# talmolab/VNL-Brax-Imitation

Measured on AMD Instinct MI355X. Metric: env-steps/sec (whole node), rodent imitation, num_envs=4096/GPU, higher is better.
Workload: dtype f32; 1 GPU; rodent imitation rollout, single groom clip, 4096 envs/GPU: intention-policy forward (HIP) -> RodentTracking.step (5 substeps, CG 6/6) -> auto-reset on -> Transition logging (unroll 20, the 20 steps replayed as one captured hipGraph); envs_per_gpu=4096, clips=1, parallelism=env-sharded x1, no data-path collective

## Files before the change

__graft_entry__.py:

```python
from __future__ import annotations

import os
import sys

ROOT = os.path.dirname(os.path.abspath(__file__))
if ROOT not in sys.path:
    sys.path.insert(0, ROOT)


def build() -> None:
    import vnl_brax_imitation_amd
    from vnl_brax_imitation_amd.csrc import build as hip_build

    from concurrent.futures import ThreadPoolExecutor

    with ThreadPoolExecutor(5) as pool:
        futs = {v: pool.submit(hip_build.build, variant=v) for v in ("product", "spill", "noblk", "nospec", "tail")}
        paths = {v: f.result() for v, f in futs.items()}
    path = paths["product"]
    assert all(os.path.exists(p_) for p_ in paths.values()), paths
    from oracle import oracle as _oracle

    _oracle.build()
    from vnl_brax_imitation_amd import _lib

    _lib.load_library(path)
    print(f"[build] {path} ok; oracle ok")


def smoke() -> None:
    import numpy as np
    import torch

    sys.path.insert(0, os.path.join(ROOT, "tests"))
    import helpers as H
    from vnl_brax_imitation_amd.envs.rodent import RodentTracking

    assert torch.cuda.is_available(), "smoke() needs a HIP device"
    B = 256
    env = RodentTracking(H.reference_clip(), num_envs=B, device="cuda:0", **H.env_kwargs())
    rng = np.random.default_rng(0)
    sf = rng.integers(0, 235, B).astype(np.int32)
    noise = (1e-3 * rng.standard_normal((B, 74))).astype(np.float32)
    st = env.reset(start_frame=torch.from_numpy(sf), noise=torch.from_numpy(noise))
    act = np.clip(0.3 * rng.standard_normal((B, 30)), -1, 1).astype(np.float32)
    o = H.make_oracle(env, "f64")
    ost = o.env_reset(sf, noise)
    e_reset = H.scaled_err(st.pipeline_state.qacc_warmstart.cpu().numpy(), ost["qacc_warmstart"])
    e_obs = H.scaled_err(st.obs.cpu().numpy(), ost["obs"])
    import parity as P
# ... 33 lines not shown
```

vnl-brax-imitation_amd/csrc/build.py:

```python
from __future__ import annotations

import os
import subprocess
import sys

HERE = os.path.dirname(os.path.abspath(__file__))
SOURCES = ["vnl_lib.hip", "vnl_policy.hip", "vnl_ppo.hip", "vnl_domain.hip"]
DEPS = SOURCES + ["vnl_env_kernels.h", "vnl_body.h", "vnl_types.h", "vnl_policy_train.h", "../../include/vnl.h"]
OUT = os.path.join(HERE, "libvnl.so")

VARIANTS = {
    "product": ("libvnl.so", ["-DVNL_KERNEL_ATTR=__attribute__((amdgpu_waves_per_eu(2,2)))"]),
    "prof": ("libvnl_prof.so", ["-DVNL_PROFILE", "-DVNL_KERNEL_ATTR=__attribute__((amdgpu_waves_per_eu(2,2)))"]),
    "knobs": ("libvnl_knobs.so", ["-DVNL_STAGE_KNOBS", "-DVNL_KERNEL_ATTR=__attribute__((amdgpu_waves_per_eu(2,2)))"]),
    "spill": ("libvnl_spill.so", ["-DVNL_KERNEL_ATTR=__attribute__((amdgpu_waves_per_eu(4,4)))"]),
    "noblk": ("libvnl_noblk.so", ["-DVNL_NO_BLK", "-DVNL_KERNEL_ATTR=__attribute__((amdgpu_waves_per_eu(2,2)))"]),
    "tail": ("libvnl_tail.so", ["-DVNL_SOLVER_TAIL", "-DVNL_KERNEL_ATTR=__attribute__((amdgpu_waves_per_eu(2,2)))"]),
    "nospec": ("libvnl_nospec.so", ["-DVNL_NO_SPEC", "-DVNL_KERNEL_ATTR=__attribute__((amdgpu_waves_per_eu(2,2)))"]),
}
ENV_KERNELS = ("vnl_step_kernel", "vnl_reset_kernel")


def resource_usage(stderr_text: str) -> dict:
    out, name = {}, None
    for line in stderr_text.splitlines():
        if "Function Name:" in line:
            name = line.split("Function Name:")[1].split()[0]
            out[name] = {}
        elif name and "remark:" in line:
            body = line.split("remark:")[1].split("[-Rpass")[0].strip()
            key, _, val = body.rpartition(":")
            try:
                out[name][key.strip()] = int(val.strip())
            except ValueError:
                pass
    return out


def build(force: bool = False, verbose: bool = False, profile: bool = False, knobs: bool = False,
          variant: str | None = None) -> str:
    variant = variant or ("prof" if profile else ("knobs" if knobs else "product"))
    fname, defs = VARIANTS[variant]
    out = os.path.join(HERE, fname)
    deps = [os.path.join(HERE, d) for d in DEPS] + [os.path.abspath(__file__)]
    newest = max(os.path.getmtime(d) for d in deps)
    if not force and os.path.exists(out) and os.path.getmtime(out) >= newest:
        return out
    hipcc = os.environ.get("HIPCC", "/opt/rocm/bin/hipcc")
    objdir = os.path.join(HERE, "_obj", variant)
    os.makedirs(objdir, exist_ok=True)
# ... 68 lines not shown
```

vnl-brax-imitation_amd/csrc/vnl_body.h:

```cpp
#pragma once
#include <math.h>

#include "vnl_types.h"

#ifndef VNL_HD
#define VNL_HD __device__ __forceinline__
#endif

#ifndef VNL_FORKJOIN_DEFINED
#define VNL_LANES 64
#define VNL_ROWS_PER_LANE 8
#define VNL_ROWS_SMALL 5
#define VNL_CHAIN_WIDTH 8
#define VNL_ROWSETS_1 1
#define VNL_ROWSETS_2 2
#define VNL_FOR(i, n) for (int i = (int)lane; i < (n); i += VNL_LANES)
#define VNL_SERIAL if (lane == 0)
#define VNL_SYNC() __builtin_amdgcn_fence(__ATOMIC_ACQ_REL, "wavefront")
#define VNL_SYNC_GLOBAL()                                     \
  do {                                                        \
    __builtin_amdgcn_fence(__ATOMIC_ACQ_REL, "wavefront");    \
    asm volatile("s_waitcnt vmcnt(0)" ::: "memory");          \
    __builtin_amdgcn_fence(__ATOMIC_ACQ_REL, "wavefront");    \
  } while (0)
// ... 123 lines not shown
VNL_HD M3 qmat(Q4 q) {
  M3 m;
  vreal q00 = q.w * q.w, q01 = q.w * q.x, q02 = q.w * q.y, q03 = q.w * q.z;
  vreal q11 = q.x * q.x, q12 = q.x * q.y, q13 = q.x * q.z, q22 = q.y * q.y, q23 = q.y * q.z, q33 = q.z * q.z;
  m.a[0] = q00 + q11 - q22 - q33, m.a[1] = vreal(2.) * (q12 - q03), m.a[2] = vreal(2.) * (q13 + q02);
  m.a[3] = vreal(2.) * (q12 + q03), m.a[4] = q00 - q11 + q22 - q33, m.a[5] = vreal(2.) * (q23 - q01);
  m.a[6] = vreal(2.) * (q13 - q02), m.a[7] = vreal(2.) * (q23 + q01), m.a[8] = q00 - q11 - q22 + q33;
  return m;
}
VNL_HD V3 mmul(const M3& m, V3 v) {
  return V3{m.a[0] * v.x + m.a[1] * v.y + m.a[2] * v.z, m.a[3] * v.x + m.a[4] * v.y + m.a[5] * v.z,
            m.a[6] * v.x + m.a[7] * v.y + m.a[8] * v.z};
}
struct S6 {
  V3 a, l;
};
VNL_HD S6 operator+(S6 p, S6 q) { return S6{p.a + q.a, p.l + q.l}; }
VNL_HD S6 operator*(S6 p, vreal s) { return S6{p.a * s, p.l * s}; }
VNL_HD vreal dot(S6 p, S6 q) { return dot(p.a, q.a) + dot(p.l, q.l); }
VNL_HD S6 mcross(S6 u, S6 v) { return S6{cross(u.a, v.a), cross(u.l, v.a) + cross(u.a, v.l)}; }
VNL_HD S6 mcross_force(S6 v, S6 f) { return S6{cross(v.a, f.a) + cross(v.l, f.l), cross(v.a, f.l)}; }

#if defined(__HIP_DEVICE_COMPILE__)
#define VNL_CAS __attribute__((address_space(4)))
#define VNL_TO_CAS(T, p) ((const VNL_CAS T*)(unsigned long long)(p))
#define VNL_LAUNDER(p) asm volatile("" : "+s"(p))
#else
#define VNL_CAS
#define VNL_TO_CAS(T, p) ((const T*)(p))
#define VNL_LAUNDER(p)
#endif
#define MI(f) (SP::fixed ? SP::D.f : m.f)
#define LO(f) (SP::fixed ? SP::L.f : L.f)
template <class SP>
struct EnvWaveT {
  const VNL_CAS DevModel& m;
  const VNL_CAS DevEnv& ev;
  const DevState& st;
  const VNL_CAS WsLayout& L;
  vreal* s;
  unsigned e, lane;
  const VNL_CAS KernelConsts* kc;
  int* trace;
  VNL_HD EnvWaveT with_trace(int* t) const { return EnvWaveT{m, ev, st, L, s, e, lane, kc, t}; }
  VNL_HD EnvWaveT fresh() const {
    const VNL_CAS KernelConsts* k = kc;
    VNL_LAUNDER(k);
    return EnvWaveT{k->m, k->ev, st, k->L, s, e, lane, k, trace};
  }
#ifdef VNL_PROFILE
  VNL_HD void prof_begin() const {
    if (lane == 0) {
      for (int i = 0; i < VNL_NPROF; i++) s[LO(prof) + i] = 0.f;
      s[LO(prof) + VNL_NPROF] = __builtin_bit_cast(float, (unsigned)__builtin_amdgcn_s_memtime());
    }
  }
  VNL_HD void prof_end() const {
    if (lane == 0)
      for (int i = 0; i < VNL_NPROF; i++) atomicAdd(&g_vnl_prof[i], (unsigned long long)s[LO(prof) + i]);
  }
#else
  VNL_HD void prof_begin() const {}
  VNL_HD void prof_end() const {}
#endif

  VNL_HD V3 ld3(int o) const { return V3{s[o], s[o + 1], s[o + 2]}; }
  VNL_HD void st3(int o, V3 v) const { s[o] = v.x, s[o + 1] = v.y, s[o + 2] = v.z; }
  VNL_HD Q4 ld4(int o) const { return Q4{s[o], s[o + 1], s[o + 2], s[o + 3]}; }
  VNL_HD S6 ld6(int o) const { return S6{ld3(o), ld3(o + 3)}; }
  VNL_HD void st6(int o, S6 v) const { st3(o, v.a), st3(o + 3, v.l); }
  VNL_HD static V3 t3(const vreal* t, int i) { return V3{t[3 * i], t[3 * i + 1], t[3 * i + 2]}; }
  VNL_HD static Q4 t4(const vreal* t, int i) { return Q4{t[4 * i], t[4 * i + 1], t[4 * i + 2], t[4 * i + 3]}; }

  VNL_HD S6 inert_mul(int o, S6 v) const {
    vreal ixx = s[o], iyy = s[o + 1], izz = s[o + 2], ixy = s[o + 3], ixz = s[o + 4], iyz = s[o + 5];
    V3 mp = ld3(o + 6);
    vreal mass = s[o + 9];
    V3 ang = V3{ixx * v.a.x + ixy * v.a.y + ixz * v.a.z, ixy * v.a.x + iyy * v.a.y + iyz * v.a.z,
                ixz * v.a.x + iyz * v.a.y + izz * v.a.z} +
             cross(mp, v.l);
    V3 lin = v.l * mass - cross(mp, v.a);
// ... 43 lines not shown
    const vreal* x = gxpos() + 3 * b;
    return V3{x[0], x[1], x[2]};
  }
  VNL_HD Q4 gquat4(int b) const {
    const vreal* q = gxquat() + 4 * b;
    return Q4{q[0], q[1], q[2], q[3]};
  }
  VNL_HD V3 ref_point() const { return MI(root_free) ? ld3(LO(qpos)) : V3{m.root_px, m.root_py, m.root_pz}; }

  VNL_HD int anc_of(int k) const { return ((const unsigned char*)(s + LO(tab_anc)))[k]; }
  VNL_HD int madr(int d) const { return ((const unsigned short*)(s + LO(tab_madr)))[d]; }
  VNL_HD int eadr(int d) const { return ((const unsigned short*)(s + LO(tab_madr)))[MI(nv) + d]; }
  VNL_HD int depth(int d) const { return eadr(d) - madr(d); }
  VNL_HD int ndesc(int d) const { return ((const unsigned short*)(s + LO(tab_madr)))[2 * MI(nv) + d]; }
  VNL_HD int parent_of(int b) const { return ((const unsigned char*)(s + LO(tab_body)))[b]; }
  VNL_HD int dofadr_of(int b) const { return ((const unsigned char*)(s + LO(tab_body)))[MI(nbody) + b]; }
  VNL_HD int dofnum_of(int b) const { return ((const unsigned char*)(s + LO(tab_body)))[2 * MI(nbody) + b]; }
  VNL_HD int con_body(int c) const { return ((const unsigned char*)(s + LO(tab_body)))[3 * MI(nbody) + c]; }
  VNL_HD unsigned short* live_rows() const { return (unsigned short*)((int*)(s + LO(act_list)) + (MI(ncon) + 3) / 4 + 2); }
  VNL_HD int num_live_rows() const { return ((const int*)(s + LO(act_list)))[(MI(ncon) + 3) / 4 + 1]; }
  template <class F>
  VNL_HD void for_live_rows(F body) const {
    const int nl = num_live_rows();
    if (nl <= VNL_LIVE_MAX) {
      const unsigned short* lv = live_rows();
      VNL_FOR(l, nl) body((int)lv[l]);
    } else {
      VNL_FOR(r, MI(nefc)) body(r);
    }
  }
  VNL_HD int con_lastdof(int c) const { return ((const unsigned char*)(s + LO(tab_body)))[3 * MI(nbody) + MI(ncon) + c]; }
  VNL_HD int lvl_dof(int q) const { return ((const unsigned char*)(s + LO(tab_lvl)))[q]; }
  VNL_HD int lvl_start(int l) const { return ((const unsigned char*)(s + LO(tab_lvl)))[MI(nv) + l]; }
  VNL_HD int jump_of(int r, int b) const { return ((const unsigned char*)(s + LO(tab_jump)))[r * MI(nbody) + b]; }
  VNL_HD void load_tables() const {
    unsigned char* ta = (unsigned char*)(s + LO(tab_anc));
    VNL_FOR(k, MI(nM)) ta[k] = (unsigned char)m.M_anc[k];
    unsigned short* tm = (unsigned short*)(s + LO(tab_madr));
    VNL_FOR(d, MI(nv)) {
      tm[d] = (unsigned short)m.dof_Madr[d], tm[MI(nv) + d] = (unsigned short)(m.dof_Madr[d] + m.dof_depth[d]);
      tm[2 * MI(nv) + d] = (unsigned short)m.dof_ndesc[d];
    }
    unsigned char* tb = (unsigned char*)(s + LO(tab_body));
    VNL_FOR(b, MI(nbody)) {
      tb[b] = (unsigned char)m.body_parent[b];
      tb[MI(nbody) + b] = (unsigned char)m.body_dofadr[b];
      tb[2 * MI(nbody) + b] = (unsigned char)m.body_dofnum[b];
    }
    VNL_FOR(c, MI(ncon)) {
      int cb = m.cg_body[m.con_geom[c] & 0xff];
      tb[3 * MI(nbody) + c] = (unsigned char)cb;
      tb[3 * MI(nbody) + MI(ncon) + c] = (unsigned char)m.body_lastdof[cb];
    }
    unsigned char* tl = (unsigned char*)(s + LO(tab_lvl));
    VNL_FOR(q, MI(nv) + MI(max_depth) + 2) tl[q] = m.lvl_tab[q];
    unsigned char* tj = (unsigned char*)(s + LO(tab_jump));
    VNL_FOR(q, MI(jump_rounds) * MI(nbody)) tj[q] = m.jump[q];
    VNL_SYNC();
  }

  VNL_HD void kinematics() const {
    int A = LO(P), Bf = LO(P) + 7 * MI(nbody);
    auto put_pose = [&](int base, int b, V3 pos, Q4 quat) {
      st3(base + 7 * b, pos);
      s[base + 7 * b + 3] = quat.w, s[base + 7 * b + 4] = quat.x, s[base + 7 * b + 5] = quat.y, s[base + 7 * b + 6] = quat.z;
    };
    auto hinge_chain = [&](int b, V3& pos, Q4& quat) {
      const int jn = m.body_jntnum[b], ja = m.body_jntadr[b];
      for (int k = 0; k < jn; k++) {
        const int j = ja + k, qa = m.jnt_qposadr[j], da = m.jnt_dofadr[j];
        V3 jp = t3(m.jnt_pos, j), jax = t3(m.jnt_axis, j);
        V3 anchor = qrot(jp, quat) + pos;
        st6(LO(cdof) + 6 * da, S6{qrot(jax, quat), anchor});
        vreal ang = s[LO(qpos) + qa] - m.jnt_qpos0[j];
        vreal sn = sin(vreal(0.5) * ang), cs = cos(vreal(0.5) * ang);
        quat = qmul(quat, Q4{cs, jax.x * sn, jax.y * sn, jax.z * sn});
        pos = anchor - qrot(jp, quat);
      }
    };
    VNL_FOR(k, MI(nbody) - 2) {
      const int b = k + 2;
      V3 pos = t3(m.body_pos, b);
      Q4 quat = t4(m.body_quat, b);
      hinge_chain(b, pos, quat);
      put_pose(A, b, pos, quat);
    }
// ... 728 lines not shown
#pragma unroll
        for (int u = 0; u < W; u++) l[u] = ld[ST * e[u]];
        vreal p0 = vreal(0.), p1 = vreal(0.);
#pragma unroll
        for (int u = 0; u < W; u += 2) {
          p0 += i + u <= iend ? l[u] * x[u] : vreal(0.);
          p1 += i + u + 1 <= iend ? l[u + 1] * x[u + 1] : vreal(0.);
        }
        acc += p0 + p1;
      }
      s[out + a] = dmode == 1 ? acc * s[dinvb + ST * a] : (dmode == 2 ? acc / s[dinvb + ST * a] : acc);
    }
    VNL_SYNC();
  }

  template <int ST, bool COL>
  VNL_HD void blk_apply(int in, int out, int dmode, int LDb, int dinvb) const {
    const int cfg = MI(blk_cfg);
    const int trips = COL ? (cfg >> 4) & 15 : cfg & 15, steps = COL ? (cfg >> 12) & 15 : (cfg >> 8) & 15;
    const unsigned* tab = m.blk_tab + (COL ? (cfg & 15) * 64 : 0);
    constexpr int W = VNL_BLK_W, MAXT = 4;
#ifdef __HIP_DEVICE_COMPILE__
    unsigned pre[MAXT];
#pragma unroll
    for (int t = 0; t < MAXT; t++) pre[t] = t < trips ? tab[t * 64 + (int)lane] : 0u;
#endif
#pragma unroll
    for (int trip = 0; trip < MAXT; trip++) {
      if (trip >= trips) break;
      VNL_PERLANE(vreal, part);
      VNL_PERLANE(unsigned, dsc);
      VNL_FOR(l, VNL_WAVE_ITEMS(64)) {
#ifdef __HIP_DEVICE_COMPILE__
        const unsigned d = pre[trip];
#else
        const unsigned d = tab[trip * 64 + l];
#endif
        const int n = (int)(d >> 16) & 15;
        vreal l_[W], x[W];
        if constexpr (!COL) {
          const int e0 = (int)(d & 0xffffu);
          const unsigned char* an = (const unsigned char*)(s + LO(tab_anc)) + e0;
          const vreal* row = s + LDb + ST * e0;
          int j[W];
#pragma unroll
          for (int u = 0; u < W; u++) j[u] = an[u], l_[u] = row[ST * u];
#pragma unroll
          for (int u = 0; u < W; u++) x[u] = s[in + j[u]];
        } else {
          const int i0 = (int)(d & 0x7fu), da = (int)(d >> 7) & 0x3f;
          const unsigned short* ea = (const unsigned short*)(s + LO(tab_madr)) + MI(nv) + i0;
          const vreal* ld = s + LDb - ST * da;
          int e[W];
#pragma unroll
          for (int u = 0; u < W; u++) e[u] = ea[u], x[u] = s[in + i0 + u];
#pragma unroll
          for (int u = 0; u < W; u++) l_[u] = ld[ST * e[u]];
        }
        vreal p0 = vreal(0.), p1 = vreal(0.);
#pragma unroll
        for (int u = 0; u < W; u++) {
          const vreal pr = u < n ? l_[u] * x[u] : vreal(0.);
          if (u & 1) p1 += pr;
          else p0 += pr;
        }
        VNL_AT(part, l) = p0 + p1;
        VNL_AT(dsc, l) = d;
// ... 203 lines not shown
      V3 size = t3(m.cg_size, g);
      vreal dist0 = vreal(0.), dist1 = vreal(0.);
      V3 cpos0 = v3(0, 0, 0), cpos1 = v3(0, 0, 0), t1 = v3(m.t1x, m.t1y, m.t1z);
      int nc = 1;
      if (type == VNL_GEOM_CAPSULE) {
        nc = 2;
        V3 axis = V3{R.a[2], R.a[5], R.a[8]};
        V3 bv = axis - n * dot(n, axis);
        vreal bn = sqrt(dot(bv, bv));
        if (bn < vreal(0.5)) {
          bv = (vreal(-0.5) < n.y && n.y < vreal(0.5)) ? v3(vreal(0.), vreal(1.), vreal(0.)) : v3(vreal(0.), vreal(0.), vreal(1.));
        } else {
          bv = bv * (vreal(1.) / bn);
        }
        t1 = bv;
        V3 ca = gpos + axis * size.y, cb = gpos - axis * size.y;
        dist0 = dot(ca - pp, n) - size.x, dist1 = dot(cb - pp, n) - size.x;
        cpos0 = ca - n * (size.x + vreal(0.5) * dist0), cpos1 = cb - n * (size.x + vreal(0.5) * dist1);
      } else if (type == VNL_GEOM_SPHERE) {
        dist0 = dot(gpos - pp, n) - size.x;
        cpos0 = gpos - n * (size.x + vreal(0.5) * dist0);
      } else {
        V3 ln = V3{(R.a[0] * n.x + R.a[3] * n.y + R.a[6] * n.z) * size.x, (R.a[1] * n.x + R.a[4] * n.y + R.a[7] * n.z) * size.y,
                   (R.a[2] * n.x + R.a[5] * n.y + R.a[8] * n.z) * size.z};
        vreal nn = sqrt(dot(ln, ln));
        vreal inv = nn > vreal(0.) ? vreal(1.) / nn : vreal(1.);
        V3 sup = V3{-ln.x * inv * size.x, -ln.y * inv * size.y, -ln.z * inv * size.z};
        V3 pos = gpos + mmul(R, sup);
        dist0 = dot(n, pos - pp);
        cpos0 = pos - n * (dist0 * vreal(0.5));
      }
      V3 t2 = cross(n, t1);
      vreal mu = par<P_MU>(g), margin = m.cg_margin[g], invw = par<P_INVW>(g);
      S6 vel = ld6(cvel + 6 * bd);
      for (int q = 0; q < nc; q++) {
        int c = c0 + q, r0 = MI(nlimit) + 4 * c;
        vreal dist = q == 0 ? dist0 : dist1;
        V3 rel = (q == 0 ? cpos0 : cpos1) - O;
        vreal d = dist - margin;
        st3(LO(con_r) + 3 * c, rel);
        if (q == 0) st3(LO(con_t1) + 3 * g, t1);
        vreal k, b, imp;
        kbimp(m.cg_solref + 2 * g, m.cg_solimp + 5 * g, m.dt, d, k, b, imp);
        vreal Rr = fmax(invw * (vreal(1.) - imp) / imp, VNL_MINVAL);
        vreal D = d < vreal(0.) ? vreal(1.) / Rr : vreal(0.);
        V3 pv = vel.l + cross(vel.a, rel);
        vreal jn = dot(n, pv), j1 = dot(t1, pv) * mu, j2 = dot(t2, pv) * mu;
        vreal kp = k * imp * d;
        s[LO(efc_D) + r0] = D, s[LO(efc_D) + r0 + 1] = D, s[LO(efc_D) + r0 + 2] = D, s[LO(efc_D) + r0 + 3] = D;
        s[LO(Jaref) + r0] = b * (jn + j1) + kp, s[LO(Jaref) + r0 + 1] = b * (jn - j1) + kp;
        s[LO(Jaref) + r0 + 2] = b * (jn + j2) + kp, s[LO(Jaref) + r0 + 3] = b * (jn - j2) + kp;
      }
    }
    VNL_SYNC();
    {
      unsigned char* act = (unsigned char*)(s + LO(act_list));
      int na = 0;
      VNL_FOR(c, VNL_PAD_ITEMS(MI(ncon))) {
        const bool on = c < MI(ncon) && s[LO(efc_D) + MI(nlimit) + 4 * (c < MI(ncon) ? c : 0)] != vreal(0.);
        int pos;
        VNL_RANK(on, na, pos);
        if (on) act[pos] = (unsigned char)c;
      }
      VNL_SERIAL { ((int*)(s + LO(act_list)))[(MI(ncon) + 3) / 4] = na; }
    }
    VNL_FOR(r, MI(nefc)) s[LO(jv) + r] = vreal(0.);
// ... 6 lines not shown
        VNL_RANK(on, nl, pos);
        if (on && pos < VNL_LIVE_MAX) lv[pos] = (unsigned short)r;
      }
      VNL_SERIAL { ((int*)(s + LO(act_list)))[(MI(ncon) + 3) / 4 + 1] = nl; }
    }
    VNL_SYNC();
    if (trace) {
      VNL_SERIAL {
        for (int w = 0; w < 16; w++) {
          int bits = 0;
          for (int b = 0; b < 32; b++) {
            const int r = 32 * w + b;
            if (r < MI(nefc) && s[LO(efc_D) + r] != vreal(0.)) bits |= 1 << b;
          }
          trace[VNL_TRACE_ROWS + w] = bits;
        }
      }
    }
  }

  VNL_HD void dof_prefix(int vec, int Q) const {
    S6 run = S6{v3(0, 0, 0), v3(0, 0, 0)}, carry = run;
    VNL_FOR(d, VNL_PAD_ITEMS(MI(nv))) {
      S6 x = S6{v3(0, 0, 0), v3(0, 0, 0)};
      if (d < MI(nv)) x = ld6(LO(cdof) + 6 * d) * s[vec + d];
      VNL_SCAN_ADD_C(x.a.x, run.a.x, carry.a.x), VNL_SCAN_ADD_C(x.a.y, run.a.y, carry.a.y);
      VNL_SCAN_ADD_C(x.a.z, run.a.z, carry.a.z), VNL_SCAN_ADD_C(x.l.x, run.l.x, carry.l.x);
      VNL_SCAN_ADD_C(x.l.y, run.l.y, carry.l.y), VNL_SCAN_ADD_C(x.l.z, run.l.z, carry.l.z);
      if (d < MI(nv)) st6(Q + 6 * (d + 1), x);
      if (d == 0) st6(Q, S6{v3(0, 0, 0), v3(0, 0, 0)});
    }
    VNL_SYNC();
  }
  VNL_HD S6 path_sum(int Q, const int* seg) const {
    S6 acc = S6{v3(0, 0, 0), v3(0, 0, 0)};
#pragma unroll
    for (int k = 0; k < 4; k++) {
      if (k >= MI(path_runs)) break;
      const int sg = seg[k], b = sg & 0xff, e = sg >> 8;
      S6 qe = ld6(Q + 6 * e), qb = ld6(Q + 6 * b);
      acc = S6{acc.a + (qe.a - qb.a), acc.l + (qe.l - qb.l)};
    }
    return acc;
  }

  VNL_HD void jac_mul(int vec, int out, bool accumulate) const {
    V3 n = v3(m.pnx, m.pny, m.pnz);
    for_live_rows([&](int r) {
      if (r < MI(nlimit)) {
        vreal v = copysign(vreal(1.), s[LO(efc_D) + r]) * s[vec + m.lim_dof[r]];
        s[out + r] = accumulate ? s[out + r] + v : v;
      }
    });
    const int Q = LO(P) + 3 * MI(nefc);
    dof_prefix(vec, Q);
    const unsigned char* act = (const unsigned char*)(s + LO(act_list));
    int na = ((const int*)(s + LO(act_list)))[(MI(ncon) + 3) / 4];
    VNL_FOR(j, na) {
      int c = act[j], g = m.con_geom[c] & 0xff, r0 = MI(nlimit) + 4 * c;
      const int* seg = m.body_pathseg + 8 * con_body(c);
      S6 vel = path_sum(Q, seg);
      vreal mu = par<P_MU>(g);
      V3 rel = ld3(LO(con_r) + 3 * c), t1 = ld3(LO(con_t1) + 3 * g), t2 = cross(n, t1);
      V3 pv = vel.l + cross(vel.a, rel);
      vreal jn = dot(n, pv), j1 = dot(t1, pv) * mu, j2 = dot(t2, pv) * mu;
      vreal o0 = jn + j1, o1 = jn - j1, o2 = jn + j2, o3 = jn - j2;
      if (accumulate) o0 += s[out + r0], o1 += s[out + r0 + 1], o2 += s[out + r0 + 2], o3 += s[out + r0 + 3];
      s[out + r0] = o0, s[out + r0 + 1] = o1, s[out + r0 + 2] = o2, s[out + r0 + 3] = o3;
    }
    VNL_SYNC();
  }

  VNL_HD vreal constraint_cost(int jaref) const {
    vreal c = vreal(0.);
    for_live_rows([&](int r) {
      vreal x = s[jaref + r];
      c += x < vreal(0.) ? fabs(s[LO(efc_D) + r]) * x * x : vreal(0.);
    });
    return vreal(0.5) * vnl_wave_sum(c);
  }

  VNL_HD vreal constraint_force() const {
    V3 n = v3(m.pnx, m.pny, m.pnz);
    int Wc = LO(P) + 3 * MI(nefc);
    vreal cost = vreal(0.);
    for_live_rows([&](int r) {
      if (r < MI(nlimit)) {
        vreal x = s[LO(Jaref) + r];
        cost += x < vreal(0.) ? fabs(s[LO(efc_D) + r]) * x * x : vreal(0.);
      }
    });
    {
      S6 run = S6{v3(0, 0, 0), v3(0, 0, 0)};
      VNL_FOR(k, VNL_WAVE_ITEMS(MI(ncon))) {
        S6 w = S6{v3(0, 0, 0), v3(0, 0, 0)};
        if (k < MI(ncon)) {
          const int c = (m.con_geom[k] >> 8) & 0xff;
          int r0 = MI(nlimit) + 4 * c;
          vreal D = s[LO(efc_D) + r0];
          if (D != vreal(0.)) {
            int g = m.con_geom[c] & 0xff;
            vreal mu = par<P_MU>(g), f[4];
            for (int q = 0; q < 4; q++) {
              vreal x = s[LO(Jaref) + r0 + q];
              f[q] = x < vreal(0.) ? -D * x : vreal(0.);
              cost += x < vreal(0.) ? D * x * x : vreal(0.);
            }
            V3 rel = ld3(LO(con_r) + 3 * c), t1 = ld3(LO(con_t1) + 3 * g), t2 = cross(n, t1);
            V3 Fw = n * (f[0] + f[1] + f[2] + f[3]) + t1 * (mu * (f[0] - f[1])) + t2 * (mu * (f[2] - f[3]));
            w = S6{cross(rel, Fw), Fw};
          }
        }
        VNL_SCAN_ADD(w.a.x, run.a.x), VNL_SCAN_ADD(w.a.y, run.a.y), VNL_SCAN_ADD(w.a.z, run.a.z);
        VNL_SCAN_ADD(w.l.x, run.l.x), VNL_SCAN_ADD(w.l.y, run.l.y), VNL_SCAN_ADD(w.l.z, run.l.z);
        if (k < MI(ncon)) st6(Wc + 6 * (k + 1), w);
        if (k == 0) st6(Wc, S6{v3(0, 0, 0), v3(0, 0, 0)});
      }
      VNL_SYNC();
      VNL_FOR(d, MI(nv)) {
        const int pk = m.dof_limrow[d], r = (pk & 0x3ff) - 1, c0 = (pk >> 10) & 0xff, c1 = (pk >> 18) & 0xff;
        S6 p1 = ld6(Wc + 6 * c1), p0 = ld6(Wc + 6 * c0);
        S6 w = S6{p1.a - p0.a, p1.l - p0.l};
        vreal q = dot(ld6(LO(cdof) + 6 * d), w);
        if (r >= 0) {
          vreal x = s[LO(Jaref) + r];
          q += x < vreal(0.) ? -s[LO(efc_D) + r] * x : vreal(0.);
        }
        s[LO(qfrc_c) + d] = q;
      }
      VNL_SYNC();
      return vreal(0.5) * vnl_wave_sum(cost);
    }
    return vreal(0.);
  }

  VNL_HD vreal vdot(int a, int b) const {
    vreal p = vreal(0.);
    VNL_FOR(d, MI(nv)) p += s[a + d] * s[b + d];
    return vnl_wave_sum(p);
  }

  struct LsPoint {
    vreal alpha, cost, d0, d1;
  };
  template <int RPL>
  struct LsRows {
    vreal ja[RPL], jv[RPL], a0[RPL], a1[RPL], a2[RPL];
  };
  template <int RPL>
  VNL_HD int ls_count_active(const LsRows<RPL>& R, vreal alpha, bool compact) const {
    int n = 0;
#pragma unroll
    for (int j = 0; j < RPL; j++) {
// ... 366 lines not shown
        const vreal* g2 = fac2();
        VNL_FOR(k, MI(nM) + MI(nv)) s[LO(P) + k] = g2[k];
        VNL_SYNC();
        solve_inplace(LO(tmp), LO(P), LO(P) + MI(nM));
      } else if (m.dbg_stage == 18) {
        tree_accumulate(LO(P), 10);
      } else if (m.dbg_stage == 19) {
        body_inertias(false);
      }
    }
#endif
    fresh().kinematics();
    VNL_PROF(0);
    fresh().body_inertias(true);
    VNL_PROF(1);
    int cvel = fresh().bias_forces();
    if (factor_pair_ok()) {
      if (MI(solver_newton)) fresh().mass_matrix(vreal(0.));
      else fresh().tree_accumulate(LO(P), 10);
      VNL_PROF(5);
      VNL_PROF(6);
      fresh().factor_both(m.dt);
      fresh().mass_mul_factor(LO(qacc), LO(mv));
      VNL_PROF(10);
      fresh().invert_both(fac2());
    } else {
      fresh().mass_matrix(vreal(0.));
      fresh().factor();
      fresh().mass_mul_factor(LO(qacc), LO(mv));
      VNL_PROF(10);
      fresh().invert_factor();
    }
    VNL_PROF(11);
    fresh().smooth_forces();
    VNL_PROF(12);
    fresh().make_constraint(cvel);
    VNL_PROF(13);
#ifdef VNL_STAGE_KNOBS
    for (int rep = 0; rep < m.dbg_count; rep++) {
      if (m.dbg_stage == 6) {
        jac_mul(LO(qacc_smooth), LO(jv), false);
      } else if (m.dbg_stage == 7) {
        VNL_FOR(d, MI(nv)) s[LO(tmp) + d] = s[LO(smooth) + d];
        VNL_SYNC();
        solve_inplace(LO(tmp));
      } else if (m.dbg_stage == 8) {
        vreal a3[3] = {vreal(0.), vreal(1e-4), vreal(2e-4)};
        LsPoint p[3];
        LsRows<VNL_ROWS_SMALL> rows;
        ls_load(rows, false);
        ls_eval<3>(rows, a3, vreal(0.), vreal(0.), vreal(0.), p);
        if (p[0].cost == vreal(-1.)) s[LO(tmp)] = p[1].cost;
      } else if (m.dbg_stage == 9) {
        make_constraint(cvel);
      } else if (m.dbg_stage == 10) {
        vreal c = constraint_force();
        if (c == vreal(-1.)) s[LO(tmp)] = c;
      } else if (m.dbg_stage == 11) {
        smooth_forces();
      } else if (m.dbg_stage == 12) {
        vreal c = vdot(LO(smooth), LO(qacc_smooth)) + vdot(LO(qacc), LO(smooth)) + vdot(LO(qacc), LO(qacc)) + vdot(LO(smooth), LO(smooth));
        if (c == vreal(-1.)) s[LO(tmp)] = c;
      } else if (m.dbg_stage == 13) {
        LsRows<VNL_ROWS_SMALL> rows;
        ls_load(rows, false);
        vreal a1[1] = {vreal(1e-4)};
        LsPoint p;
        ls_eval<1>(rows, a1, vreal(0.), vreal(0.), vreal(0.), &p);
        if (p.cost == vreal(-1.)) s[LO(tmp)] = p.cost;
      }
    }
#endif
    fresh().solve();
  }

  VNL_HD void euler() const {
    const int nv = MI(nv);
    VNL_PROF(26);
    VNL_FOR(d, nv) s[LO(tmp) + d] = MI(eulerdamp) ? s[LO(smooth) + d] + s[LO(qfrc_c) + d] : s[LO(qacc) + d];
    VNL_SYNC();
    if (MI(eulerdamp) && factor_pair_ok()) {
      const vreal* g2 = fac2();
      const int n2 = MI(nM) + MI(nv);
      VNL_SYNC_GLOBAL();
      VNL_FOR(k, n2) s[LO(P) + k] = g2[k];
      VNL_SYNC();
      fresh().solve_inplace(LO(tmp), LO(P), LO(P) + MI(nM));
      VNL_PROF(27);
    } else if (MI(eulerdamp)) {
      fresh().body_inertias(false);
      VNL_PROF(1);
      fresh().mass_matrix(m.dt);
      fresh().factor();
      fresh().invert_factor();
      fresh().solve_inplace(LO(tmp));
      VNL_PROF(27);
    }
    VNL_FOR(i, MI(nu)) {
      if (m.act_tau[i] >= vreal(0.)) s[LO(act) + i] += s[LO(actdot) + i] * m.dt;
    }
    VNL_FOR(d, nv) s[LO(qvel) + d] += s[LO(tmp) + d] * m.dt;
    VNL_SYNC();
    VNL_FOR(j, MI(njnt)) {
      int qa = m.jnt_qposadr[j], da = m.jnt_dofadr[j];
      if (m.jnt_type[j] == VNL_JNT_FREE) {
        for (int t = 0; t < 3; t++) s[LO(qpos) + qa + t] += m.dt * s[LO(qvel) + da + t];
        V3 w = ld3(LO(qvel) + da + 3);
        vreal nrm = sqrt(dot(w, w));
        V3 ax = nrm > vreal(0.) ? w * (vreal(1.) / nrm) : w;
        vreal ang = m.dt * nrm, sn = sin(vreal(0.5) * ang), cs = cos(vreal(0.5) * ang);
        Q4 r = qmul(ld4(LO(qpos) + qa + 3), Q4{cs, ax.x * sn, ax.y * sn, ax.z * sn});
        vreal n2 = sqrt(r.w * r.w + r.x * r.x + r.y * r.y + r.z * r.z);
        vreal inv = n2 > vreal(0.) ? vreal(1.) / n2 : vreal(1.);
        s[LO(qpos) + qa + 3] = r.w * inv, s[LO(qpos) + qa + 4] = r.x * inv, s[LO(qpos) + qa + 5] = r.y * inv,
                        s[LO(qpos) + qa + 6] = r.z * inv;
      } else {
        s[LO(qpos) + qa] += m.dt * s[LO(qvel) + da];
      }
    }
    VNL_SYNC();
    VNL_PROF(28);
  }

  VNL_HD static int clampi(int v, int lo, int hi) { return v < lo ? lo : (v > hi ? hi : v); }
  VNL_HD static vreal nan0(vreal x) {
    if (x != x) return vreal(0.);
    if (x > vreal(3.4028235e38)) return vreal(3.4028235e38);
    if (x < -vreal(3.4028235e38)) return -vreal(3.4028235e38);
// ... 279 lines not shown
```

vnl-brax-imitation_amd/csrc/vnl_lib.hip:

```cpp
#include <hip/hip_runtime.h>
#include <stdint.h>
#include <stdio.h>
#include <stdlib.h>
#include <string.h>

#include <algorithm>
#include <cmath>
#include <cstddef>
#include <map>
#include <string>
#include <vector>

#include "../../include/vnl.h"
#include "vnl_body.h"

static thread_local char g_err[512] = "";
static int fail(int code, const char* fmt, const char* a = "", const char* b = "") {
  snprintf(g_err, sizeof(g_err), fmt, a, b);
  return code;
}
#define HIPCHK(call)                                                              \
  do {                                                                            \
    hipError_t e_ = (call);                                                       \
    if (e_ != hipSuccess) return fail(VNL_ERR_HIP, "%s: %s", #call, hipGetErrorString(e_)); \
// ... 730 lines not shown
      if (I("jnt_limited")[j] && I("jnt_type")[j] == VNL_JNT_HINGE) {
        const int dd = I("jnt_dofadr")[j];
        if (dd < 0 || dd >= nv || ++nlim[dd] > 1)
          return fail(VNL_ERR_UNSUPPORTED, "Newton solver: a limit row does not act on exactly one dof of its own");
      }
    for (int g = 0; g < ng; g++) {
      const int b = I("cg_bodyid")[g];
      if (b < 0 || b >= nb) return fail(VNL_ERR_UNSUPPORTED, "Newton solver: a contact is not attached to one dynamic body");
    }
    if (((d.fac_route >> VNL_ROUTE_QM_INVERSE) & 0xf) == VNL_ROUTE_LDS)
      return fail(VNL_ERR_UNSUPPORTED, "Newton solver: dof tree too deep for the register-resident inversion of the "
                                       "Hessian's factor (max depth < 36; rows 64 .. of depth < 16; nv <= 128)");
  }
  return VNL_OK;
}

static void layout(vnl_env* env) {
  const DevModel& d = env->dm;
  const WsLayout L = vnl_make_layout(dims_of(d));
  env->L = L;
  auto sec = [&](const char* name, int at, int n) { env->sections[name] = {at, n}; };
  sec("qpos", L.qpos, d.nq), sec("qvel", L.qvel, d.nv), sec("act", L.act, d.nu), sec("ctrl", L.ctrl, d.nu);
  sec("act_dot", L.actdot, d.nu), sec("subtree_com1", L.com, 4), sec("cdof", L.cdof, 6 * d.nv);
  sec("qLD", L.LD, L.dinv - L.LD), sec("qLDiagInv", L.dinv, d.nv), sec("pool", L.P, L.smooth - L.P);
  sec("efc_D", L.efc_D, d.nefc), sec("Jaref", L.Jaref, d.nefc), sec("jv", L.jv, d.nefc);
  sec("qfrc_smooth", L.smooth, d.nv), sec("qacc_smooth", L.qacc_smooth, d.nv), sec("qacc", L.qacc, d.nv);
  sec("Ma", L.Ma, d.nv), sec("grad", L.grad, d.nv), sec("Mgrad", L.Mgrad, d.nv), sec("search", L.search, d.nv);
  sec("mv", L.mv, d.nv), sec("qfrc_constraint", L.qfrc_c, d.nv), sec("tmp", L.tmp, d.nv), sec("tmp2", L.tmp2, d.nv);
  sec("con_r", L.con_r, 3 * d.ncon), sec("con_t1", L.con_t1, 3 * d.ncg);
  sec("tab_anc", L.tab_anc, L.tab_madr - L.tab_anc), sec("tab_madr", L.tab_madr, L.tab_body - L.tab_madr);
  sec("tab_body", L.tab_body, L.tab_jump - L.tab_body), sec("tab_jump", L.tab_jump, L.tab_lvl - L.tab_jump);
  sec("tab_lvl", L.tab_lvl, L.act_list - L.tab_lvl);
  sec("act_list", L.act_list, vnl_words(4 * (long)((d.ncon + 3) / 4) + 8 + 2 * VNL_LIVE_MAX));
  if (d.solver_newton) {
    sec("newton_qM", L.newt_M, d.nM), sec("newton_LD", L.newt_H, d.nM), sec("newton_LDiagInv", L.newt_H + d.nM, d.nv);
  }
#ifdef VNL_PROFILE
  sec("prof", L.prof, 2 * (VNL_NPROF + 1));
#endif
}

static bool same_layout(const WsLayout& a, const WsLayout& b) { return memcmp(&a, &b, sizeof(WsLayout)) == 0; }
static bool same_dims(const VnlDims& a, const VnlDims& b) { return memcmp(&a, &b, sizeof(VnlDims)) == 0; }

#include "vnl_env_kernels.h"

extern "C" void vnl_env_destroy(vnl_env* env) {
  if (!env) return;
  for (void* p : env->allocs) (void)hipFree(p);
  delete env->fmap;
  delete env;
}

extern "C" int vnl_env_create(const vnl_model* hm, const vnl_envspec* es, int32_t num_envs, int32_t device,
                              vnl_env** out) {
  if (!hm || !es || !out || num_envs <= 0) return fail(VNL_ERR_ARG, "vnl_env_create: bad argument");
  int ndev = 0;
  if (hipGetDeviceCount(&ndev) != hipSuccess || ndev <= 0)
    return fail(VNL_ERR_NO_DEVICE, "no HIP device: the rollout has no CPU fallback");
  if (device < 0 || device >= ndev) return fail(VNL_ERR_ARG, "device ordinal out of range");
  DeviceGuard guard(device);
  if (!guard.ok) return fail(VNL_ERR_HIP, "hipSetDevice failed");
  vnl_env* env = new vnl_env();
  env->device = device, env->B = num_envs;
  int rc = build_dev_model(env, hm);
  if (rc != VNL_OK) {
    vnl_env_destroy(env);
    return rc;
  }
  const DevModel& d = env->dm;
  DevEnv& e = env->de;
  e.T = es->clip_frames, e.C = es->num_clips, e.ref_len = es->ref_traj_length, e.sub_clip_length = es->sub_clip_length;
  e.n_frames = es->n_frames, e.nb = es->num_track_bodies, e.nee = es->num_end_eff, e.napp = es->num_appendages;
  e.njc = es->num_joint_cols, e.com_ref_col = es->com_ref_col;
  e.healthy_lo = es->healthy_z_lo, e.healthy_hi = es->healthy_z_hi;
  e.inv_term_threshold = vreal(1) / es->termination_threshold, e.body_err_mult = es->body_error_multiplier;
// ... 779 lines not shown
```

vnl-brax-imitation_amd/csrc/vnl_types.h:

```cpp
#pragma once
#include <stdint.h>

#ifndef VNL_REAL
#define VNL_REAL float
#endif
typedef VNL_REAL vreal;

#define VNL_JNT_FREE 0
#define VNL_JNT_HINGE 3
#define VNL_GEOM_SPHERE 2
#define VNL_GEOM_CAPSULE 3
#define VNL_GEOM_ELLIPSOID 4

#define VNL_TRACE_ITERS 8
#define VNL_TRACE_REC 64
#define VNL_TRACE_ROWS (8 + VNL_TRACE_REC * VNL_TRACE_ITERS)
#define VNL_TRACE_INTS (VNL_TRACE_ROWS + 16)

#define VNL_LIVE_MAX 128
#define VNL_BLK_W 13
#define VNL_FAC_LINES 6

#define VNL_ROUTE_LDS 1
#define VNL_ROUTE_ROWS16 2
// ... 44 lines not shown
  const vreal *act_gain, *act_tau, *act_lo, *act_hi, *act_gear;
  const int *cg_type, *cg_body, *cg_conadr, *cg_ncon, *con_geom;
  const vreal *cg_pos, *cg_quat, *cg_size, *cg_mu, *cg_solref, *cg_solimp, *cg_margin, *cg_invweight;
};

struct DevEnv {
  int T, C, ref_len, sub_clip_length, n_frames, nb, nee, napp, njc, com_ref_col;
  int obs_size, traj_size;
  int flags;
  vreal healthy_lo, healthy_hi, inv_term_threshold, body_err_mult, done_threshold;
  vreal w_reward[6];
  const int *body_idxs, *end_eff_idx, *app_body, *app_ref_col, *joint_cols;
  const float *position, *quaternion, *joints, *body_positions, *velocity, *angular_velocity, *joints_velocity;
  const float* center_of_mass;
  vreal* fac2;
};

struct DevState {
  vreal *qpos, *qvel, *act, *warm, *xpos, *xquat, *com1, *qfrc_actuator;
  vreal *obs, *reward, *done, *metrics, *traj, *term_err;
  int *cur_frame, *sub_clip_frame, *clip_id;
};

struct WsLayout {
  int qpos, qvel, act, ctrl, actdot, com;
  int cdof, LD, dinv;
  int P;
  int efc_D, Jaref, jv;
  int smooth, qacc_smooth, qacc, Ma, grad, Mgrad, search, mv, qfrc_c, tmp, tmp2;
  int prof;
  int con_r, con_t1;
  int tab_anc, tab_madr, tab_body, tab_jump, tab_lvl;
  int act_list;
  int newt_M, newt_H;
  int total;
};

struct VnlDims {
  int nq, nv, nu, nbody, njnt, ncg, ncon, nlimit, nefc, nM;
  int iterations, ls_iterations, eulerdamp, root_free, max_depth, jump_rounds, fac_steps, fac_route, solver_newton, blk_cfg, path_runs, nbody_out;
};

#ifndef VNL_NPROF_SLOTS
#ifdef VNL_PROFILE
#define VNL_NPROF_SLOTS (2 * (40 + 1))
#else
#define VNL_NPROF_SLOTS 0
#endif
#endif
constexpr int vnl_imax(int a, int b) { return a > b ? a : b; }
constexpr int vnl_words(long bytes) { return (int)((bytes + (long)sizeof(vreal) - 1) / (long)sizeof(vreal)); }
constexpr WsLayout vnl_make_layout(const VnlDims& d) {
  WsLayout L{};
  int o = 0;
  auto sec = [&o](int n) {
    int at = o;
    o += n;
    return at;
  };
  L.qpos = sec(d.nq), L.qvel = sec(d.nv), L.act = sec(d.nu), L.ctrl = sec(d.nu);
  L.actdot = sec(d.nu), L.com = sec(4);
  L.cdof = sec(6 * d.nv);
  L.LD = sec(vnl_imax(d.nM, 6 * (d.nv + 1) + 6 * (d.nbody + 1)));
  L.dinv = sec(d.nv);
  int pool = vnl_imax(vnl_imax(14 * d.nbody, 22 * d.nbody), 3 * d.nefc + vnl_imax(6 * (d.ncon + 1), 6 * (d.nv + 1)));
  if (d.eulerdamp) pool = vnl_imax(pool, d.nM + d.nv);
  L.P = sec(pool);
  L.efc_D = L.P, L.Jaref = L.P + d.nefc, L.jv = L.P + 2 * d.nefc;
  L.smooth = sec(d.nv), L.qacc_smooth = sec(d.nv), L.qacc = sec(d.nv);
  L.Ma = sec(d.nv), L.grad = sec(d.nv), L.Mgrad = sec(d.nv), L.search = sec(d.nv);
  L.mv = sec(d.nv), L.qfrc_c = sec(d.nv), L.tmp = sec(d.nv), L.tmp2 = sec(d.nv);
  L.con_r = sec(3 * d.ncon), L.con_t1 = sec(3 * d.ncg);
  L.tab_anc = sec(vnl_words(d.nM)), L.tab_madr = sec(vnl_words(6 * (long)d.nv));
  L.tab_body = sec(vnl_words(3 * (long)d.nbody + 2 * (long)d.ncon));
  L.tab_jump = sec(vnl_words((long)(d.jump_rounds > 0 ? d.jump_rounds : 1) * d.nbody));
  L.tab_lvl = sec(vnl_words((long)d.nv + d.max_depth + 2));
  L.act_list = sec(vnl_words(4 * (long)((d.ncon + 3) / 4) + 8 + 2 * VNL_LIVE_MAX));
  L.newt_M = L.newt_H = 0;
  if (d.solver_newton) L.newt_M = sec(d.nM), L.newt_H = sec(d.nM + d.nv);
  if (VNL_NPROF_SLOTS) {
    o = (o + 1) & ~1;
    L.prof = sec(VNL_NPROF_SLOTS);
  }
  L.total = (o + 3) & ~3;
  return L;
}

constexpr int vnl_vstore(int P) { return (P + 3) & ~3; }
constexpr int vnl_cvel_at(int P, int smooth, int nbody, int nv) {
  const int a = P + 16 * nbody, b = vnl_vstore(P) + 12 * nv;
  return (b > a && b + 6 * nbody <= smooth) ? b : a;
}

struct VnlSpecGeneric {
  static constexpr bool fixed = false;
  static constexpr bool dom = false;
  static constexpr VnlDims D{};
  static constexpr WsLayout L{};
};
struct VnlSpecRodent {
  static constexpr bool fixed = true;
  static constexpr bool dom = false;
  static constexpr VnlDims D{74, 73, 30, 53, 68, 32, 59, 67, 303, 1119, 6, 6, 1, 1, 35, 5, 36,
                             VNL_ROUTE_ROWS36X2 | (VNL_ROUTE_ROWS36X2 << VNL_ROUTE_QM_INVERSE) | (2 << VNL_ROUTE_PAIR), 0,
                             2 | (2 << 4) | (2 << 8) | (3 << 12), 2, 66};
  static constexpr WsLayout L = vnl_make_layout(D);
};
template <class BASE>
struct VnlSpecDom : BASE {
  static constexpr bool dom = true;
// ... 18 lines not shown
```

Baseline: 2.518 million env-steps/s.

## Stage solver lookup tables in LDS and hoist block/limit tables into registers

Adds per-env LDS tables for contact geom indices, ordered contacts, path runs, limit dofs and friction coefficients, filled once in load_tables and make_constraint, so the CG solve's jac_mul and transpose loops read LDS instead of global model arrays. It also preloads the block-factor table and per-dof limit-row words into VGPRs before smooth_forces, make_constraint and solve, and keeps them live with asm barriers. The aim is to remove repeated global and scalar loads from the inner solver iterations. The cost is more LDS per workgroup, which a static_assert caps at the 8-workgroups-per-CU limit, plus extra register pressure under waves_per_eu(2,2). A 'plain' build variant keeps the old path for comparison.

```diff
diff --git a/__graft_entry__.py b/__graft_entry__.py
--- a/__graft_entry__.py
+++ b/__graft_entry__.py
@@ -14,8 +14,8 @@
 
     from concurrent.futures import ThreadPoolExecutor
 
-    with ThreadPoolExecutor(5) as pool:
-        futs = {v: pool.submit(hip_build.build, variant=v) for v in ("product", "spill", "noblk", "nospec", "tail")}
+    with ThreadPoolExecutor(6) as pool:
+        futs = {v: pool.submit(hip_build.build, variant=v) for v in ("product", "spill", "noblk", "nospec", "tail", "plain")}
         paths = {v: f.result() for v, f in futs.items()}
     path = paths["product"]
     assert all(os.path.exists(p_) for p_ in paths.values()), paths
diff --git a/vnl-brax-imitation_amd/csrc/build.py b/vnl-brax-imitation_amd/csrc/build.py
--- a/vnl-brax-imitation_amd/csrc/build.py
+++ b/vnl-brax-imitation_amd/csrc/build.py
@@ -16,6 +16,7 @@
     "spill": ("libvnl_spill.so", ["-DVNL_KERNEL_ATTR=__attribute__((amdgpu_waves_per_eu(4,4)))"]),
     "noblk": ("libvnl_noblk.so", ["-DVNL_NO_BLK", "-DVNL_KERNEL_ATTR=__attribute__((amdgpu_waves_per_eu(2,2)))"]),
     "tail": ("libvnl_tail.so", ["-DVNL_SOLVER_TAIL", "-DVNL_KERNEL_ATTR=__attribute__((amdgpu_waves_per_eu(2,2)))"]),
+    "plain": ("libvnl_plain.so", ["-DVNL_SOLVER_PLAIN", "-DVNL_KERNEL_ATTR=__attribute__((amdgpu_waves_per_eu(2,2)))"]),
     "nospec": ("libvnl_nospec.so", ["-DVNL_NO_SPEC", "-DVNL_KERNEL_ATTR=__attribute__((amdgpu_waves_per_eu(2,2)))"]),
 }
 ENV_KERNELS = ("vnl_step_kernel", "vnl_reset_kernel")
diff --git a/vnl-brax-imitation_amd/csrc/vnl_body.h b/vnl-brax-imitation_amd/csrc/vnl_body.h
--- a/vnl-brax-imitation_amd/csrc/vnl_body.h
+++ b/vnl-brax-imitation_amd/csrc/vnl_body.h
@@ -179,6 +179,20 @@
 #endif
 #define MI(f) (SP::fixed ? SP::D.f : m.f)
 #define LO(f) (SP::fixed ? SP::L.f : L.f)
+#if defined(__HIP_DEVICE_COMPILE__) && !defined(VNL_SOLVER_PLAIN)
+#define VNL_SOLVE_REGS 1
+#else
+#define VNL_SOLVE_REGS 0
+#endif
+#define VNL_BLK_REGS 2
+#define VNL_LIMROW_REGS 2
+#define VNL_SR_BLK 1
+#define VNL_SR_LIMROW 2
+struct VnlSolveRegs {
+  int on;
+  unsigned blk[2][VNL_BLK_REGS];
+  int limrow[VNL_LIMROW_REGS];
+};
 template <class SP>
 struct EnvWaveT {
   const VNL_CAS DevModel& m;
@@ -189,11 +203,44 @@
   unsigned e, lane;
   const VNL_CAS KernelConsts* kc;
   int* trace;
-  VNL_HD EnvWaveT with_trace(int* t) const { return EnvWaveT{m, ev, st, L, s, e, lane, kc, t}; }
+  VnlSolveRegs sr;
+  VNL_HD EnvWaveT with_trace(int* t) const { return EnvWaveT{m, ev, st, L, s, e, lane, kc, t, sr}; }
   VNL_HD EnvWaveT fresh() const {
     const VNL_CAS KernelConsts* k = kc;
     VNL_LAUNDER(k);
-    return EnvWaveT{k->m, k->ev, st, k->L, s, e, lane, k, trace};
+    return EnvWaveT{k->m, k->ev, st, k->L, s, e, lane, k, trace, sr};
+  }
+  VNL_HD EnvWaveT with_solve_regs(bool with_limrow) const {
+    EnvWaveT w = *this;
+#if VNL_SOLVE_REGS
+    const int cfg = MI(blk_cfg), tr = cfg & 15, tc = (cfg >> 4) & 15;
+    const bool blk = blk_on();
+#pragma unroll
+    for (int t = 0; t < VNL_BLK_REGS; t++) {
+      w.sr.blk[0][t] = (blk && t < tr) ? m.blk_tab[t * 64 + (int)lane] : 0u;
+      w.sr.blk[1][t] = (blk && t < tc) ? m.blk_tab[(tr + t) * 64 + (int)lane] : 0u;
+    }
+#pragma unroll
+    for (int q = 0; q < VNL_LIMROW_REGS; q++) {
+      const int d = (int)lane + 64 * q;
+      w.sr.limrow[q] = (with_limrow && d < MI(nv)) ? m.dof_limrow[d] : 0;
+    }
+#pragma unroll
+    for (int t = 0; t < VNL_BLK_REGS; t++) asm volatile("" : "+v"(w.sr.blk[0][t]), "+v"(w.sr.blk[1][t]));
+    if (with_limrow) {
+#pragma unroll
+      for (int q = 0; q < VNL_LIMROW_REGS; q++) asm volatile("" : "+v"(w.sr.limrow[q]));
+    }
+    w.sr.on = with_limrow ? (VNL_SR_BLK | VNL_SR_LIMROW) : VNL_SR_BLK;
+#endif
+    return w;
+  }
+  VNL_HD int limrow_of(int d) const {
+#if VNL_SOLVE_REGS
+    static_assert(VNL_LIMROW_REGS == 2, "limrow_of selects between exactly two registers");
+    if ((sr.on & VNL_SR_LIMROW) && d < 64 * VNL_LIMROW_REGS) return d < 64 ? sr.limrow[0] : sr.limrow[1];
+#endif
+    return m.dof_limrow[d];
   }
 #ifdef VNL_PROFILE
   VNL_HD void prof_begin() const {
@@ -303,6 +350,19 @@
   VNL_HD int con_lastdof(int c) const { return ((const unsigned char*)(s + LO(tab_body)))[3 * MI(nbody) + MI(ncon) + c]; }
   VNL_HD int lvl_dof(int q) const { return ((const unsigned char*)(s + LO(tab_lvl)))[q]; }
   VNL_HD int lvl_start(int l) const { return ((const unsigned char*)(s + LO(tab_lvl)))[MI(nv) + l]; }
+#ifndef VNL_SOLVER_PLAIN
+  VNL_HD int con_geom_of(int c) const { return ((const unsigned char*)(s + LO(tab_con)))[2 * c]; }
+  VNL_HD int con_ordered(int k) const { return ((const unsigned char*)(s + LO(tab_con)))[2 * k + 1]; }
+  VNL_HD int lim_dof_of(int r) const { return ((const unsigned char*)(s + LO(tab_lim)))[r]; }
+  VNL_HD int con_path_run(int c, int k) const { return ((const unsigned short*)(s + LO(tab_path)))[c * MI(path_runs) + k]; }
+  VNL_HD vreal con_mu_of(int g) const { return s[LO(con_mu) + g]; }
+#else
+  VNL_HD int con_geom_of(int c) const { return m.con_geom[c] & 0xff; }
+  VNL_HD int con_ordered(int k) const { return (m.con_geom[k] >> 8) & 0xff; }
+  VNL_HD int lim_dof_of(int r) const { return m.lim_dof[r]; }
+  VNL_HD int con_path_run(int c, int k) const { return m.body_pathseg[8 * con_body(c) + k]; }
+  VNL_HD vreal con_mu_of(int g) const { return par<P_MU>(g); }
+#endif
   VNL_HD int jump_of(int r, int b) const { return ((const unsigned char*)(s + LO(tab_jump)))[r * MI(nbody) + b]; }
   VNL_HD void load_tables() const {
     unsigned char* ta = (unsigned char*)(s + LO(tab_anc));
@@ -318,11 +378,18 @@
       tb[MI(nbody) + b] = (unsigned char)m.body_dofadr[b];
       tb[2 * MI(nbody) + b] = (unsigned char)m.body_dofnum[b];
     }
+    unsigned char* tc = (unsigned char*)(s + LO(tab_con));
+    unsigned short* tp = (unsigned short*)(s + LO(tab_path));
     VNL_FOR(c, MI(ncon)) {
-      int cb = m.cg_body[m.con_geom[c] & 0xff];
+      const int cg = m.con_geom[c];
+      int cb = m.cg_body[cg & 0xff];
       tb[3 * MI(nbody) + c] = (unsigned char)cb;
       tb[3 * MI(nbody) + MI(ncon) + c] = (unsigned char)m.body_lastdof[cb];
-    }
+      tc[2 * c] = (unsigned char)(cg & 0xff), tc[2 * c + 1] = (unsigned char)((cg >> 8) & 0xff);
+      for (int k = 0; k < MI(path_runs); k++) tp[c * MI(path_runs) + k] = (unsigned short)m.body_pathseg[8 * cb + k];
+    }
+    unsigned char* tlim = (unsigned char*)(s + LO(tab_lim));
+    VNL_FOR(r, MI(nlimit)) tlim[r] = (unsigned char)m.lim_dof[r];
     unsigned char* tl = (unsigned char*)(s + LO(tab_lvl));
     VNL_FOR(q, MI(nv) + MI(max_depth) + 2) tl[q] = m.lvl_tab[q];
     unsigned char* tj = (unsigned char*)(s + LO(tab_jump));
@@ -1117,7 +1184,7 @@
       VNL_PERLANE(unsigned, dsc);
       VNL_FOR(l, VNL_WAVE_ITEMS(64)) {
 #ifdef __HIP_DEVICE_COMPILE__
-        const unsigned d = pre[trip];
+        const unsigned d = (VNL_SOLVE_REGS && (sr.on & VNL_SR_BLK) && trip < VNL_BLK_REGS) ? sr.blk[COL ? 1 : 0][trip] : pre[trip];
 #else
         const unsigned d = tab[trip * 64 + l];
 #endif
@@ -1387,6 +1454,7 @@
       }
       V3 t2 = cross(n, t1);
       vreal mu = par<P_MU>(g), margin = m.cg_margin[g], invw = par<P_INVW>(g);
+      s[LO(con_mu) + g] = mu;
       S6 vel = ld6(cvel + 6 * bd);
       for (int q = 0; q < nc; q++) {
         int c = c0 + q, r0 = MI(nlimit) + 4 * c;
@@ -1459,23 +1527,26 @@
     }
     VNL_SYNC();
   }
-  VNL_HD S6 path_sum(int Q, const int* seg) const {
+  template <class RUN>
+  VNL_HD S6 path_sum_runs(int Q, RUN run) const {
     S6 acc = S6{v3(0, 0, 0), v3(0, 0, 0)};
 #pragma unroll
     for (int k = 0; k < 4; k++) {
       if (k >= MI(path_runs)) break;
-      const int sg = seg[k], b = sg & 0xff, e = sg >> 8;
+      const int sg = run(k), b = sg & 0xff, e = sg >> 8;
       S6 qe = ld6(Q + 6 * e), qb = ld6(Q + 6 * b);
       acc = S6{acc.a + (qe.a - qb.a), acc.l + (qe.l - qb.l)};
     }
     return acc;
   }
+  VNL_HD S6 path_sum(int Q, const int* seg) const { return path_sum_runs(Q, [&](int k) { return seg[k]; }); }
+  VNL_HD S6 path_sum_con(int Q, int c) const { return path_sum_runs(Q, [&](int k) { return con_path_run(c, k); }); }
 
   VNL_HD void jac_mul(int vec, int out, bool accumulate) const {
     V3 n = v3(m.pnx, m.pny, m.pnz);
     for_live_rows([&](int r) {
       if (r < MI(nlimit)) {
-        vreal v = copysign(vreal(1.), s[LO(efc_D) + r]) * s[vec + m.lim_dof[r]];
+        vreal v = copysign(vreal(1.), s[LO(efc_D) + r]) * s[vec + lim_dof_of(r)];
         s[out + r] = accumulate ? s[out + r] + v : v;
       }
     });
@@ -1484,10 +1555,9 @@
     const unsigned char* act = (const unsigned char*)(s + LO(act_list));
     int na = ((const int*)(s + LO(act_list)))[(MI(ncon) + 3) / 4];
     VNL_FOR(j, na) {
-      int c = act[j], g = m.con_geom[c] & 0xff, r0 = MI(nlimit) + 4 * c;
-      const int* seg = m.body_pathseg + 8 * con_body(c);
-      S6 vel = path_sum(Q, seg);
-      vreal mu = par<P_MU>(g);
+      int c = act[j], g = con_geom_of(c), r0 = MI(nlimit) + 4 * c;
+      S6 vel = path_sum_con(Q, c);
+      vreal mu = con_mu_of(g);
       V3 rel = ld3(LO(con_r) + 3 * c), t1 = ld3(LO(con_t1) + 3 * g), t2 = cross(n, t1);
       V3 pv = vel.l + cross(vel.a, rel);
       vreal jn = dot(n, pv), j1 = dot(t1, pv) * mu, j2 = dot(t2, pv) * mu;
@@ -1522,12 +1592,12 @@
       VNL_FOR(k, VNL_WAVE_ITEMS(MI(ncon))) {
         S6 w = S6{v3(0, 0, 0), v3(0, 0, 0)};
         if (k < MI(ncon)) {
-          const int c = (m.con_geom[k] >> 8) & 0xff;
+          const int c = con_ordered(k);
           int r0 = MI(nlimit) + 4 * c;
           vreal D = s[LO(efc_D) + r0];
           if (D != vreal(0.)) {
-            int g = m.con_geom[c] & 0xff;
-            vreal mu = par<P_MU>(g), f[4];
+            int g = con_geom_of(c);
+            vreal mu = con_mu_of(g), f[4];
             for (int q = 0; q < 4; q++) {
               vreal x = s[LO(Jaref) + r0 + q];
               f[q] = x < vreal(0.) ? -D * x : vreal(0.);
@@ -1545,7 +1615,7 @@
       }
       VNL_SYNC();
       VNL_FOR(d, MI(nv)) {
-        const int pk = m.dof_limrow[d], r = (pk & 0x3ff) - 1, c0 = (pk >> 10) & 0xff, c1 = (pk >> 18) & 0xff;
+        const int pk = limrow_of(d), r = (pk & 0x3ff) - 1, c0 = (pk >> 10) & 0xff, c1 = (pk >> 18) & 0xff;
         S6 p1 = ld6(Wc + 6 * c1), p0 = ld6(Wc + 6 * c0);
         S6 w = S6{p1.a - p0.a, p1.l - p0.l};
         vreal q = dot(ld6(LO(cdof) + 6 * d), w);
@@ -1978,9 +2048,10 @@
       fresh().invert_factor();
     }
     VNL_PROF(11);
-    fresh().smooth_forces();
+    const EnvWaveT w = fresh().with_solve_regs(true);
+    w.smooth_forces();
     VNL_PROF(12);
-    fresh().make_constraint(cvel);
+    w.make_constraint(cvel);
     VNL_PROF(13);
 #ifdef VNL_STAGE_KNOBS
     for (int rep = 0; rep < m.dbg_count; rep++) {
@@ -2017,7 +2088,7 @@
       }
     }
 #endif
-    fresh().solve();
+    w.solve();
   }
 
   VNL_HD void euler() const {
@@ -2031,7 +2102,7 @@
       VNL_SYNC_GLOBAL();
       VNL_FOR(k, n2) s[LO(P) + k] = g2[k];
       VNL_SYNC();
-      fresh().solve_inplace(LO(tmp), LO(P), LO(P) + MI(nM));
+      fresh().with_solve_regs(false).solve_inplace(LO(tmp), LO(P), LO(P) + MI(nM));
       VNL_PROF(27);
     } else if (MI(eulerdamp)) {
       fresh().body_inertias(false);
@@ -2039,7 +2110,7 @@
       fresh().mass_matrix(m.dt);
       fresh().factor();
       fresh().invert_factor();
-      fresh().solve_inplace(LO(tmp));
+      fresh().with_solve_regs(false).solve_inplace(LO(tmp));
       VNL_PROF(27);
     }
     VNL_FOR(i, MI(nu)) {
diff --git a/vnl-brax-imitation_amd/csrc/vnl_lib.hip b/vnl-brax-imitation_amd/csrc/vnl_lib.hip
--- a/vnl-brax-imitation_amd/csrc/vnl_lib.hip
+++ b/vnl-brax-imitation_amd/csrc/vnl_lib.hip
@@ -786,6 +786,8 @@
   sec("tab_body", L.tab_body, L.tab_jump - L.tab_body), sec("tab_jump", L.tab_jump, L.tab_lvl - L.tab_jump);
   sec("tab_lvl", L.tab_lvl, L.act_list - L.tab_lvl);
   sec("act_list", L.act_list, vnl_words(4 * (long)((d.ncon + 3) / 4) + 8 + 2 * VNL_LIVE_MAX));
+  sec("tab_con", L.tab_con, L.tab_path - L.tab_con), sec("tab_path", L.tab_path, L.tab_lim - L.tab_path);
+  sec("tab_lim", L.tab_lim, L.con_mu - L.tab_lim), sec("con_mu", L.con_mu, d.ncg);
   if (d.solver_newton) {
     sec("newton_qM", L.newt_M, d.nM), sec("newton_LD", L.newt_H, d.nM), sec("newton_LDiagInv", L.newt_H + d.nM, d.nv);
   }
@@ -796,6 +798,9 @@
 
 static bool same_layout(const WsLayout& a, const WsLayout& b) { return memcmp(&a, &b, sizeof(WsLayout)) == 0; }
 static bool same_dims(const VnlDims& a, const VnlDims& b) { return memcmp(&a, &b, sizeof(VnlDims)) == 0; }
+#ifndef VNL_PROFILE
+static_assert(sizeof(vreal) != 4 || (size_t)VnlSpecRodent::L.total * sizeof(vreal) <= 20480, "the rodent's LDS layout no longer allows 8 workgroups per CU");
+#endif
 
 #include "vnl_env_kernels.h"
 
diff --git a/vnl-brax-imitation_amd/csrc/vnl_types.h b/vnl-brax-imitation_amd/csrc/vnl_types.h
--- a/vnl-brax-imitation_amd/csrc/vnl_types.h
+++ b/vnl-brax-imitation_amd/csrc/vnl_types.h
@@ -100,6 +100,7 @@
   int con_r, con_t1;
   int tab_anc, tab_madr, tab_body, tab_jump, tab_lvl;
   int act_list;
+  int tab_con, tab_path, tab_lim, con_mu;
   int newt_M, newt_H;
   int total;
 };
@@ -144,6 +145,8 @@
   L.tab_jump = sec(vnl_words((long)(d.jump_rounds > 0 ? d.jump_rounds : 1) * d.nbody));
   L.tab_lvl = sec(vnl_words((long)d.nv + d.max_depth + 2));
   L.act_list = sec(vnl_words(4 * (long)((d.ncon + 3) / 4) + 8 + 2 * VNL_LIVE_MAX));
+  L.tab_con = sec(vnl_words(2 * (long)d.ncon)), L.tab_path = sec(vnl_words(2 * (long)d.path_runs * d.ncon));
+  L.tab_lim = sec(vnl_words(d.nlimit)), L.con_mu = sec(d.ncg);
   L.newt_M = L.newt_H = 0;
   if (d.solver_newton) L.newt_M = sec(d.nM), L.newt_H = sec(d.nM + d.nv);
   if (VNL_NPROF_SLOTS) {
```

New measurement: 2.549 million env-steps/s, median of 6. 1.01x the previous value.
